# kocvara/Loraine.jl

Measured on AMD Instinct MI355X. Metric: ms/IP-iteration (Schur assembly + solve), dense SDP n=2000 m=4000, lower is better.
Workload: dtype f64; 1 GPU; C4 synthetic dense SDP, matrix side 2000, 4000 constraints, kit=0 (assembly + Cholesky + predictor/corrector solves); msz=2000, nvar=4000, seed=20250614, parallelism=1 GPU

## Files before the change

### loraine.jl_amd/csrc/api.hip

```cpp
#include <cstring>

#include "../../include/loraine_hip.h"
#include "ctx.h"

using namespace lrn;

void lrn_free_model(lrn_ctx* c);
namespace lrn {
void prec_free(lrn_ctx* c);
}

extern "C" {

int lrn_version(void) { return 102; }

int lrn_device_count(void) {
  int n = 0;
  if (hipGetDeviceCount(&n) != hipSuccess) {
    (void)hipGetLastError();
    return 0;
  }
  return n;
}

// ... 58 lines not shown
}

int lrn_set_option(lrn_ctx* c, const char* key, double value) {
  if (!c || !key) return LRN_ERR_ARG;
  if (!strcmp(key, "dense_threshold")) c->opt.dense_threshold = value;
  else if (!strcmp(key, "profile")) c->profile = value != 0.0;
  else if (!strcmp(key, "t_batch")) { c->opt.t_batch = (long)value; for (auto& b : c->lmi) b.t_cap = b.p_cap = 0; }
  else if (!strcmp(key, "p_batch")) { c->opt.p_batch = (long)value; for (auto& b : c->lmi) b.t_cap = b.p_cap = 0; }
  else if (!strcmp(key, "prec_eig")) c->opt.prec_eig = (int)value;
  else if (!strcmp(key, "pivot_boost")) c->opt.pivot_boost = value;
  else if (!strcmp(key, "schur_chol")) c->opt.schur_chol = (int)value;
  else if (!strcmp(key, "schur_plan")) c->opt.schur_plan = (int)value;
  else if (!strcmp(key, "gemm3_ksplit")) c->opt.gemm3_ksplit = (int)value;
  else if (!strcmp(key, "gemm_no_skip")) c->opt.gemm_no_skip = (int)value;
  else if (!strcmp(key, "gemm_dyn_masks")) c->opt.gemm_dyn_masks = (int)value;
  else if (!strcmp(key, "gemm1_diag")) c->opt.gemm1_diag = (int)value;
  else if (!strcmp(key, "gemm_lab")) c->opt.gemm_lab = (int)value & 127;
  else if (!strcmp(key, "gemm3_sched")) c->opt.gemm3_sched = (int)value;
  else if (!strcmp(key, "gemm3_tile")) c->opt.gemm3_tile = (int)value;
  else if (!strcmp(key, "gemm3_strip")) c->opt.gemm3_strip = (int)value;
  else if (!strcmp(key, "gemm3_stagger")) c->opt.gemm3_stagger = (int)value;
  else if (!strcmp(key, "jacobi_wgs")) c->opt.jacobi_wgs = (int)value;
  else if (!strcmp(key, "jacobi_block")) c->opt.jacobi_block = (int)value;
  else if (!strcmp(key, "jacobi_inner")) c->opt.jacobi_inner = (int)value;
  else if (!strcmp(key, "pair_lanes")) c->opt.pair_lanes = (int)value;
  else if (!strcmp(key, "matvec_sparse")) c->opt.matvec_sparse = (int)value;
  else if (!strcmp(key, "prec_dense")) c->opt.prec_dense = (int)value;
  else if (!strcmp(key, "wmw_pattern_min")) c->opt.wmw_pattern_min = std::max(2, (int)value);
  else if (!strcmp(key, "profile_symv")) c->opt.profile_symv = (int)value;
  else if (!strcmp(key, "profile_ops")) c->opt.profile_ops = (int)value;
// ... 461 lines not shown
```

### loraine.jl_amd/csrc/ctx.h

```cpp
#pragma once
#include <map>

#include "chol.h"
#include "lrn_common.h"

namespace lrn { struct Prec; struct Comm; }

struct LmiBlock {
  int msz = 0;
  long nent = 0;
  std::vector<int> sigma;
  std::vector<int> ipos;
  std::vector<long> nnz;
  int qA = 0;
  int nd = 0;
  int q_wave = 0;
  int npos_nz = 0;
  long p_cap = 0, t_cap = 0;
  lrn::DBuf ent_ptr;
  lrn::DBuf ent_r, ent_c;
  lrn::DBuf ent_v;
  lrn::DBuf Adense;
  int dense_sym = -1;
  lrn::DBuf tri_tab;
// ... 34 lines not shown
  bool factored = false;
};

struct lrn_ctx;
namespace lrn { void update_shard_bs(lrn_ctx* c); }

struct LrnOptions {
  double dense_threshold = -1.0;
  long t_batch = 0, p_batch = 0;
  int prec_eig = 0;
  double pivot_boost = 1e-12;
  int schur_chol = -1;
  int schur_plan = -1;
  int gemm3_ksplit = 0;
  int gemm_dyn_masks = 0;
  int gemm_lab = 0;
  int gemm1_diag = 1;
  int gemm_no_skip = 0;
  int gemm3_sched = 1;
  int gemm3_strip = 1;
  int gemm3_tile = 0;
  int gemm3_stagger = 0;
  int jacobi_inner = 0;
  int jacobi_wgs = 0;
  int jacobi_block = 0;
  int jacobi_cross = 1;
  int prepw_streams = 1;
  int lz_resident = 1;
  int eigmin_pair = 2;
  double jacobi_early = 3e-8;
// ... 133 lines not shown
```

### loraine.jl_amd/csrc/gemm_f64.hip

```cpp
#include "lrn_common.h"

#include <algorithm>
#include <map>
#include <mutex>
#include <type_traits>
#include <utility>
#include <vector>

namespace lrn {

static constexpr int BK = 16;
static constexpr int MAX_KSPLIT = 64;

struct GemmParams {
  GemmDesc d;
  int tilesM, tilesN;
  int kchunk;
  int kcols[MAX_KSPLIT + 1];
  int kcols2[MAX_KSPLIT + 1];
  const int2* tile_list;
  const int2* tile_list2;
  int n1, n2;
  int m_org = 0, n_org = 0;
};

#define MFMA_F64_ROW(lane, r) (((lane) >> 4) + 4 * (r))
#define LRN_MFMA_INPLACE(c, a, b) asm volatile("v_mfma_f64_16x16x4_f64 %0, %1, %2, %0" : "+v"(c) : "v"(a), "v"(b))
#define LRN_MFMA_DRAIN() asm volatile("s_nop 15\n\ts_nop 15\n\ts_nop 15" ::: "memory")

template <int BM, bool KC>
__device__ __forceinline__ int lds_idx(int m, int k) {
  return KC ? (m * (BK + 2) + k) : (k * (BM + 16) + m);
}

template <int BM, int BN, bool AKC, bool BKC, bool KSEG, bool EPI>
__global__ __launch_bounds__(256, 2) void gemm_f64_kernel(GemmParams p) {
  constexpr int TM = BM / 32, TN = BN / 32;
  constexpr int EA = BM * BK / 256, EB = BN * BK / 256;
  constexpr int LA = BK * (BM + 16), LB = BK * (BN + 16);
  __shared__ double lds[2 * (LA + LB)];

  const GemmDesc& d = p.d;
  int tm, tn;
// ... 200 lines not shown
          *c = v;
          if (mir) Cg[(long)n * d.sCm + (long)m * d.sCn] = v;
          if (EPI && d.C2) d.C2[(long)n * d.sCm + (long)m * d.sCn] = v;
        }
      }
}

template <int BM, int BN, bool KSEG, bool EPI>
static void launch4(hipStream_t st, const GemmParams& p, bool akc, bool bkc, dim3 grid) {
  if (akc && bkc) hipLaunchKernelGGL((gemm_f64_kernel<BM, BN, true, true, KSEG, EPI>), grid, dim3(256), 0, st, p);
  else if (akc) hipLaunchKernelGGL((gemm_f64_kernel<BM, BN, true, false, KSEG, EPI>), grid, dim3(256), 0, st, p);
  else if (bkc) hipLaunchKernelGGL((gemm_f64_kernel<BM, BN, false, true, KSEG, EPI>), grid, dim3(256), 0, st, p);
  else hipLaunchKernelGGL((gemm_f64_kernel<BM, BN, false, false, KSEG, EPI>), grid, dim3(256), 0, st, p);
}

template <bool EPI, bool DYN>
__global__ __launch_bounds__(256, 2) void gemm_f64_lds_kernel(GemmParams p) {
  constexpr int BM = 128, BN = 128, TM = 4, TN = 4;
  constexpr int LROW = BM + 16;
  constexpr int LA = BK * LROW;
  __shared__ double lds[2 * 2 * LA];
  const GemmDesc& d = p.d;
  int tm, tn;
  {
    int bid = blockIdx.x, nwg = gridDim.x;
    int q = nwg >> 3, r = nwg & 7, xcd = bid & 7;
    int swz = (xcd < r ? xcd * (q + 1) : r * (q + 1) + (xcd - r) * q) + (bid >> 3);
    if ((d.flags & (GEMM_KFROM_N | GEMM_KFROM_M | GEMM_KTO_N | GEMM_KTO_M)) && r == 0) {
      xcd = (xcd + (int)blockIdx.z) & 7;
      swz = xcd * q + (bid >> 3);
    }
// ... 77 lines not shown
#pragma unroll
    for (int kk = 0; kk < BK / 4; ++kk) {
      double fa[TM], fb[TN];
#pragma unroll
      for (int i = 0; i < TM; ++i) fa[i] = sa[(kk * 4 + fk) * LROW + (2 * i + wm) * 16 + fr];
#pragma unroll
      for (int j = 0; j < TN; ++j) fb[j] = sb[(kk * 4 + fk) * LROW + (2 * j + wn) * 16 + fr];
#pragma unroll
      for (int i = 0; i < TM; ++i)
#pragma unroll
        for (int j = 0; j < TN; ++j)
          acc[i][j] = __builtin_amdgcn_mfma_f64_16x16x4f64(fa[i], fb[j], acc[i][j], 0, 0, 0);
    }
    __syncthreads();
  };
  auto step_mask = [&](int kt) __attribute__((always_inline)) -> unsigned {
    unsigned mask = smask;
    const int sn = kt - n0 / BK, sm = kt - m0 / BK;
#pragma unroll
    for (int j = 0; j < TN; ++j) {
      const int bn = 2 * j + wn;
      if ((from_n && sn < bn) || (to_n && sn > bn)) mask &= ~(0x1111u << j);
    }
#pragma unroll
    for (int i = 0; i < TM; ++i) {
      const int bm = 2 * i + wm;
      if ((from_m && sm < bm) || (to_m && sm > bm)) mask &= ~(0xfu << (4 * i));
    }
    return mask;
  };
// ... 91 lines not shown
      else if ((smask & ~0xf731u) == 0u) e[10] = nk;
      else if ((smask & ~0x7777u) == 0u) e[3] = nk;
      else if ((smask & ~0x0fffu) == 0u) e[6] = nk;
    }
#define LRN_PATTERN_LOOP(q, m)                                                             \
    {                                                                                      \
      const int end = e[q] < nk ? e[q] : nk;                                               \
      for (; kt < end; ++kt) static_step(std::integral_constant<unsigned, m>{}, kt);       \
    }
    LRN_PATTERN_LOOP(0, 0x0000u)
    LRN_PATTERN_LOOP(1, 0x1111u) LRN_PATTERN_LOOP(2, 0x3333u) LRN_PATTERN_LOOP(3, 0x7777u)
    LRN_PATTERN_LOOP(4, 0x000fu) LRN_PATTERN_LOOP(5, 0x00ffu) LRN_PATTERN_LOOP(6, 0x0fffu)
    LRN_PATTERN_LOOP(7, 0x08ceu) LRN_PATTERN_LOOP(8, 0x8cefu)
    LRN_PATTERN_LOOP(9, 0x7310u) LRN_PATTERN_LOOP(10, 0xf731u)
#undef LRN_PATTERN_LOOP
    for (; kt < nk; ++kt) fast_step(kt);
  }
  LRN_MFMA_DRAIN();
  if (d.flags & GEMM_LAB_NO_STORE) return;

  const bool x2 = EPI && (d.flags & GEMM_OFFDIAG_X2) && (tm != tn);
  const double alpha = x2 ? 2.0 * d.alpha : d.alpha;
  const bool sq = EPI && (d.flags & GEMM_SQUARE);
  const bool pk = EPI && (d.flags & GEMM_C_PACKED);
  const bool mir = EPI && (d.flags & GEMM_C_MIRROR) && (tm != tn);
  const int pkS = packed_S(d.pk_m);
  const long pkKd = packed_diag_elems(d.pk_m > 0 ? d.pk_m : 1);
  if (pk && !sq) {
    const long S16 = pkS >> 4, kd16 = pkKd >> 4;
    const int qb = (m0 + d.pk_off) >> 4, rbb = (n0 + d.pk_off) >> 4;
#pragma unroll
// ... 145 lines not shown
  if (trace && t == 0) trace[6] = wall_clock64();
  double* __restrict__ Cg = d.C + (long)ks * d.sCs;
#pragma unroll
  for (int i = 0; i < 2; ++i)
#pragma unroll
    for (int j = 0; j < 2; ++j)
#pragma unroll
      for (int r = 0; r < 4; ++r) {
        const int m = m0 + wm * 32 + i * 16 + MFMA_F64_ROW(lane, r);
        const int n = n0 + wn * 32 + j * 16 + fr;
        if (m < d.M && n < d.N) Cg[(long)m * d.sCm + n] = d.alpha * acc[i][j][r];
      }
  if (trace && t == 0) trace[7] = wall_clock64();
}

template <bool FLAT, int TBM, int TBN>
__global__ __launch_bounds__(256, 2) void gemm_f64_kseg_lds_kernel(GemmParams p) {
  constexpr int BM = 32 * TBM, BN = 32 * TBN, TM = TBM, TN = TBN;
  constexpr int LA = BM * BK, LB = BN * BK;
  extern __shared__ double lds[];
  const GemmDesc& d = p.d;
  int tm, tn, ks, bz;
  if (p.n2 >= 0) {
    const int xcd = blockIdx.x & 7, l = blockIdx.x >> 3;
    const int q1 = p.n1 >> 3, q2 = p.n2 >> 3;
    int2 tt;
    if (l < d.ksplit * q1) { ks = l / q1; tt = p.tile_list[xcd * q1 + l % q1]; }
    else { const int l2 = l - d.ksplit * q1; ks = l2 / q2; tt = p.tile_list2[xcd * q2 + l2 % q2]; }
    tm = tt.x;
    tn = tt.y;
    bz = 0;
// ... 86 lines not shown
      for (int j = 0; j < TN; ++j) {
        const int bm = 2 * i + wm, bn = 2 * j + wn;
        bool need = (m0 + 16 * bm < d.M) && (n0 + 16 * bn < d.N);
        if ((diag_lo && bm < bn) || (diag_up && bn < bm)) need = false;
        if (d.flags & GEMM_NO_SKIP) need = true;
        if (need) smask |= 1u << (i * TN + j);
      }
  }
  bool more = FLAT ? left > 0 : segc < segcend;
  if (more) {
    issue(chunk_base(), 0);
    next_chunk();
  }
  __syncthreads();
  int cur = 0;
  if (smask == (1u << (TM * TN)) - 1u) {
    while (more) {
      const bool have_next = FLAT ? left > 0 : segc < segcend;
      if (have_next) {
        issue(chunk_base(), cur ^ 1);
        next_chunk();
      }
      const double* sa = lds + cur * (LA + LB);
      const double* sb = same_panel ? sa : sa + LA;
#pragma unroll
      for (int kk = 0; kk < BK / 4; ++kk) {
        double fa[TM], fb[TN];
        const int k = kk * 4 + fk;
#pragma unroll
        for (int i = 0; i < TM; ++i) {
          int row = (2 * i + wm) * 16 + fr;
// ... 61 lines not shown
        int m = m0 + (2 * i + wm) * 16 + MFMA_F64_ROW(lane, r);
        int n = n0 + (2 * j + wn) * 16 + fr;
        if (m < d.M && n < d.N) Cg[(long)m * d.sCm + (long)n * d.sCn] = d.alpha * acc[i][j][r];
      }
    }
}

static bool kseg_lds_path_ok(const GemmDesc& d) {
  if (d.sAk != 1 || d.sBk != 1 || d.beta != 0.0) return false;
  if ((d.flags & GEMM_KFLAT) ? ((d.kflat_total & 15) || (d.kflat_diag & 15)) : (d.kseg_ld & 15)) return false;
  if ((d.sAm & 1) || (d.sBn & 1) || (d.bA & 1) || (d.bB & 1)) return false;
  if (((uintptr_t)d.A & 15) || ((uintptr_t)d.B & 15)) return false;
  if (d.flags & (GEMM_OFFDIAG_X2 | GEMM_SQUARE | GEMM_SQUARE_BLOCKSUM)) return false;
  return true;
}

static bool lds_path_ok(const GemmDesc& d) {
  if (d.sAm != 1 || d.sBn != 1 || d.ksplit != 1) return false;
  if (d.flags & GEMM_SQUARE_BLOCKSUM) return false;
  static const bool aligned_only = getenv("LRN_LDS_ALIGNED") != nullptr;
  if (d.sAk < d.M || d.sBk < d.N || (aligned_only && ((d.sAk & 1) || (d.sBk & 1)))) return false;
  if (aligned_only && (((uintptr_t)d.A & 15) || ((uintptr_t)d.B & 15) || (d.bA & 1) || (d.bB & 1))) return false;
  if (d.K < 256) return false;
  if ((double)d.K * (double)d.sAk * 8.0 >= 2.0e9 || (double)d.K * (double)d.sBk * 8.0 >= 2.0e9) return false;
  return true;
}

static const int2* get_tile_list(int tilesM, int tilesN, int tri, int* count, int short_sel = 0, bool edge_m = false,
                                 bool edge_n = false, bool diag = false, int korder = 0) {
  struct Key {
// ... 52 lines not shown
}

static thread_local const char* tls_gemm_error = nullptr;
const char* gemm_last_error() { return tls_gemm_error; }
static int gemm_fail(int code, const char* why) { tls_gemm_error = why; return code; }

static int gemm_impl(hipStream_t st, const GemmDesc& din);
static bool big_tile_attr_ok() {
  static bool done[64] = {false}, ok[64] = {false};
  int dev = 0;
  if (hipGetDevice(&dev) != hipSuccess || dev < 0 || dev >= 64) return false;
  if (!done[dev]) {
    ok[dev] = hipFuncSetAttribute((const void*)gemm_f64_kseg_lds_kernel<true, 5, 5>,
                                  hipFuncAttributeMaxDynamicSharedMemorySize, 2 * 2 * 160 * BK * 8) == hipSuccess &&
              hipFuncSetAttribute((const void*)gemm_f64_kseg_lds_kernel<true, 4, 5>,
                                  hipFuncAttributeMaxDynamicSharedMemorySize, 2 * (128 + 160) * BK * 8) == hipSuccess;
    done[dev] = true;
  }
  return ok[dev];
}

#include <map>
#include <mutex>
static double* split_slabs(hipStream_t st, size_t bytes) {
  static std::mutex mu;
  static std::map<std::pair<int, hipStream_t>, std::pair<void*, size_t>> cache;
  int dev = 0;
  if (hipGetDevice(&dev) != hipSuccess) return nullptr;
  std::lock_guard<std::mutex> lk(mu);
  auto& e = cache[{dev, st}];
// ... 51 lines not shown
        out->p = slabs; out->stride = (long)mn; out->n = ks;
        return LRN_OK;
      }
      if (out) { out->p = din.C; out->stride = 0; out->n = 1; }
      return reduce_slabs(st, slabs, (long)mn, ks, din.C, (long)mn, din.beta);
    }
  }
  if (out) { out->p = din.C; out->stride = 0; out->n = 1; }
  const int rc = gemm_impl(st, din);
  if (rc != LRN_OK && !tls_gemm_error) tls_gemm_error = "kernel launch failed";
  return rc;
}

int gemm(hipStream_t st, const GemmDesc& din) { return gemm_maybe_slabs(st, din, nullptr); }
int gemm_slabs(hipStream_t st, const GemmDesc& din, SlabSrc* out) { return gemm_maybe_slabs(st, din, out); }

static int gemm_impl(hipStream_t st, const GemmDesc& din) {
  GemmParams p;
  p.d = din;
  GemmDesc& d = p.d;
  if (d.M <= 0 || d.N <= 0 || d.batch <= 0) return LRN_OK;
  if (d.ksplit < 1) d.ksplit = 1;
  if (d.ksplit > MAX_KSPLIT) return gemm_fail(LRN_ERR_ARG, "gemm: d.ksplit > MAX_KSPLIT");
  long asCm = d.sCm < 0 ? -d.sCm : d.sCm, asCn = d.sCn < 0 ? -d.sCn : d.sCn;
  bool swapped = false;
  if (asCm < asCn) {
    swapped = true;
    if (d.flags & GEMM_KFROM_N) d.flags = (d.flags & ~GEMM_KFROM_N) | GEMM_KFROM_M;
    else if (d.flags & GEMM_KFROM_M) d.flags = (d.flags & ~GEMM_KFROM_M) | GEMM_KFROM_N;
    if (d.flags & GEMM_KTO_N) d.flags = (d.flags & ~GEMM_KTO_N) | GEMM_KTO_M;
// ... 99 lines not shown
    int c1 = 0, c2 = 0;
    p.tile_list = get_tile_list(p.tilesM, p.tilesN, trif, &c1, 1, em, en, dg);
    p.tile_list2 = get_tile_list(p.tilesM, p.tilesN, trif, &c2, 2, em, en, dg);
    if (!p.tile_list || !p.tile_list2) return gemm_fail(LRN_ERR_NOMEM, "gemm: tile list allocation failed");
    p.n1 = c1;
    p.n2 = c2;
    if (c1 + c2 == 0) return LRN_OK;
    if (c1 == 0) { p.tile_list = p.tile_list2; p.n1 = c2; p.n2 = 0; }
    const long wgs = 8L * d.ksplit * ((p.n1 >> 3) + (p.n2 >> 3));
    if (wgs > 0x7fffffffL) return gemm_fail(LRN_ERR_ARG, "gemm: grid too large");
    dim3 grid1((unsigned)wgs, 1, 1);
    if (big) {
      if (!big_tile_attr_ok()) return gemm_fail(LRN_ERR_HIP, "gemm: 80 KB of dynamic LDS refused");
      hipLaunchKernelGGL((gemm_f64_kseg_lds_kernel<true, 5, 5>), grid1, dim3(256), 2 * 2 * 160 * BK * 8, st, p);
    } else {
      hipLaunchKernelGGL((gemm_f64_kseg_lds_kernel<true, 4, 4>), grid1, dim3(256), 2 * 2 * 128 * BK * 8, st, p);
    }
    return hipGetLastError() == hipSuccess ? LRN_OK : LRN_ERR_HIP;
  }
  if (d.tile_class == 4 || d.tile_class == 5) {
    const int rem = d.M % 128;
    if (!kflat || d.batch != 1 || big || d.M != d.N || rem == 0 || rem > 32 || d.M < 288 ||
        (d.flags & (GEMM_TRI_LOWER | GEMM_TRI_UPPER)) != GEMM_TRI_UPPER || !(d.flags & GEMM_DIAG_UPPER) ||
        (d.flags & GEMM_NO_SKIP))
      return gemm_fail(LRN_ERR_ARG, "gemm: tile_class 4 needs the symmetric K-contiguous update with M % 128 in (0, 32]");
    if (!big_tile_attr_ok()) return gemm_fail(LRN_ERR_HIP, "gemm: 80 KB of dynamic LDS refused");
    const int Mm = d.M - 128 - rem, tmain = Mm / 128;
    if (d.tile_class == 4) {
      GemmParams pm = p;
      pm.d.M = Mm; pm.d.N = Mm;
      pm.tilesM = tmain; pm.tilesN = tmain;
      int c1 = 0, c2 = 0;
      pm.tile_list = get_tile_list(tmain, tmain, GEMM_TRI_UPPER, &c1, 1, false, false, true);
      pm.tile_list2 = get_tile_list(tmain, tmain, GEMM_TRI_UPPER, &c2, 2, false, false, true);
      if (!pm.tile_list || !pm.tile_list2) return gemm_fail(LRN_ERR_NOMEM, "gemm: tile list allocation failed");
      pm.n1 = c1;
      pm.n2 = c2;
      if (c1 == 0) { pm.tile_list = pm.tile_list2; pm.n1 = c2; pm.n2 = 0; }
      const long wgs = 8L * d.ksplit * ((pm.n1 >> 3) + (pm.n2 >> 3));
      if (wgs > 0x7fffffffL) return gemm_fail(LRN_ERR_ARG, "gemm: grid too large");
      if (wgs > 0)
        hipLaunchKernelGGL((gemm_f64_kseg_lds_kernel<true, 4, 4>), dim3((unsigned)wgs, 1, 1), dim3(256),
                           2 * 2 * 128 * BK * 8, st, pm);
    } else {
      GemmParams ps = p;
      ps.d.flags &= ~(GEMM_TRI_LOWER | GEMM_TRI_UPPER | GEMM_DIAG_LOWER | GEMM_DIAG_UPPER);
      ps.m_org = 0; ps.n_org = Mm;
      ps.tilesM = tmain + 2; ps.tilesN = 1;
      int cnt = 0;
      ps.tile_list = get_tile_list(tmain + 2, 1, 0, &cnt);
      if (!ps.tile_list || cnt <= 0) return gemm_fail(LRN_ERR_NOMEM, "gemm: tile list allocation failed");
      hipLaunchKernelGGL((gemm_f64_kseg_lds_kernel<true, 4, 5>), dim3(cnt, 1, d.ksplit), dim3(256),
                         2 * (128 + 160) * BK * 8, st, ps);
    }
    return hipGetLastError() == hipSuccess ? LRN_OK : gemm_fail(LRN_ERR_HIP, "gemm: launch failed");
  }
  static const int tile_order = getenv("LRN_TILE_ORDER") ? atoi(getenv("LRN_TILE_ORDER")) : 0;
  const int korder = (tile_order && d.tile_class == 0 && d.batch > 1) ? ((d.flags & GEMM_KFROM_N) ? 1 : (d.flags & GEMM_KFROM_M) ? 2 : 0) : 0;
  p.tile_list = get_tile_list(p.tilesM, p.tilesN, d.flags & (GEMM_TRI_LOWER | GEMM_TRI_UPPER), &ntile, d.tile_class,
                              d.tile_class != 0 && (d.M % BMv) != 0, d.tile_class != 0 && (d.N % BMv) != 0,
                              d.tile_class != 0 && (d.flags & (GEMM_DIAG_LOWER | GEMM_DIAG_UPPER)) != 0, korder);
  if (d.tile_class != 0 && p.tile_list && ntile == 0) return LRN_OK;
  if (!p.tile_list || ntile <= 0) return gemm_fail(LRN_ERR_NOMEM, "gemm: tile list allocation failed");
  (void)tri;
  const bool akc = (d.sAk == 1 && d.sAm != 1);
  const bool bkc = (d.sBk == 1 && d.sBn != 1);
  dim3 grid(ntile, 1, d.batch * d.ksplit);
  if (grid.z > 65535) return gemm_fail(LRN_ERR_ARG, "gemm: grid.z > 65535");
  const bool epi = (d.flags & (GEMM_OFFDIAG_X2 | GEMM_SQUARE | GEMM_SQUARE_BLOCKSUM | GEMM_C_PACKED | GEMM_C_MIRROR)) || d.C2;
  if (d.C2 && (d.M != d.N || d.batch != 1 || d.ksplit != 1 || kseg)) return gemm_fail(LRN_ERR_ARG, "gemm: C2 needs a square, unbatched, unsplit product");
  if (kflat) {
    if (big) {
      if (!big_tile_attr_ok()) return gemm_fail(LRN_ERR_HIP, "gemm: 80 KB of dynamic LDS refused");
      hipLaunchKernelGGL((gemm_f64_kseg_lds_kernel<true, 5, 5>), grid, dim3(256), 2 * 2 * 160 * BK * 8, st, p);
    } else {
      hipLaunchKernelGGL((gemm_f64_kseg_lds_kernel<true, 4, 4>), grid, dim3(256), 2 * 2 * 128 * BK * 8, st, p);
    }
    return hipGetLastError() == hipSuccess ? LRN_OK : LRN_ERR_HIP;
  }
  if (kseg && kseg_lds_path_ok(d)) {
    hipLaunchKernelGGL((gemm_f64_kseg_lds_kernel<false, 4, 4>), grid, dim3(256), 2 * 2 * 128 * BK * 8, st, p);
    return hipGetLastError() == hipSuccess ? LRN_OK : LRN_ERR_HIP;
  }
  if (!small && !kseg && lds_path_ok(d)) {
    const unsigned dyn = (d.flags & GEMM_LAB_ONE_WG) ? 24576u : 0u;
    if (dyn) {
      (void)hipFuncSetAttribute((const void*)gemm_f64_lds_kernel<true, false>, hipFuncAttributeMaxDynamicSharedMemorySize, (int)dyn);
      (void)hipFuncSetAttribute((const void*)gemm_f64_lds_kernel<false, false>, hipFuncAttributeMaxDynamicSharedMemorySize, (int)dyn);
    }
    if (d.flags & GEMM_DYN_MASKS) {
      if (epi) hipLaunchKernelGGL((gemm_f64_lds_kernel<true, true>), grid, dim3(256), 0, st, p);
      else hipLaunchKernelGGL((gemm_f64_lds_kernel<false, true>), grid, dim3(256), 0, st, p);
    } else {
      if (epi) hipLaunchKernelGGL((gemm_f64_lds_kernel<true, false>), grid, dim3(256), dyn, st, p);
      else hipLaunchKernelGGL((gemm_f64_lds_kernel<false, false>), grid, dim3(256), dyn, st, p);
    }
    return hipGetLastError() == hipSuccess ? LRN_OK : LRN_ERR_HIP;
  }
  if (small && mid_mode != 0 && !kseg && !epi && d.batch == 1 && d.beta == 0.0 && d.sAm == 1 && d.sBn == 1 && d.K >= 64 &&
      d.sCn == 1 && d.sAk >= d.M && d.sBk >= d.N && !(d.flags & ~(GEMM_SMALL_TILE | GEMM_TRI_LOWER | GEMM_TRI_UPPER)) &&
      (!tri || (d.M == d.N && d.ksplit > 1)) &&
      (double)d.K * (double)std::max(d.sAk, d.sBk) * 8.0 < 2.0e9) {
    static const char* trace_path = getenv("LRN_MID_TRACE");
    static int trace_launch = 0;
    unsigned long long* tb = nullptr;
    p.n1 = (tri ? p.tilesM * (p.tilesM + 1) / 2 : p.tilesM * p.tilesN) * d.ksplit;
    grid = dim3((unsigned)((p.n1 + 7) & ~7), 1, 1);
    const size_t tw = 8 * (size_t)grid.x * grid.z;
    if (trace_path && ++trace_launch == 40 && hipMalloc(&tb, tw * 8) == hipSuccess) {
      (void)hipMemsetAsync(tb, 0, tw * 8, st);
// ... 98 lines not shown
```

### loraine.jl_amd/csrc/lrn_common.h

```cpp
#pragma once
#include <hip/hip_runtime.h>

#include <cstdint>
#include <cstdio>
#include <cstring>
#include <string>
#include <vector>

#define LRN_OK 0
#define LRN_ERR_ARG (-1)
#define LRN_ERR_HIP (-2)
#define LRN_ERR_STATE (-3)
#define LRN_ERR_NOMEM (-4)

typedef double v4f64 __attribute__((ext_vector_type(4)));

namespace lrn {

__host__ __device__ inline int shard_owner(int blk, int world) {
  int r = blk % world;
  return ((blk / world) & 1) ? world - 1 - r : r;
}
__host__ __device__ inline int shard_global_block(int rank, int lb, int world) {
  return lb * world + ((lb & 1) ? world - 1 - rank : rank);
// ... 19 lines not shown
  GEMM_KTO_N = 1024,
  GEMM_KTO_M = 2048,
  GEMM_C_MIRROR = 4096,
  GEMM_DIAG_LOWER = 8192,
  GEMM_DIAG_UPPER = 16384,
  GEMM_TILE160 = 65536,
  GEMM_DYN_MASKS = 131072,
  GEMM_NO_SKIP = 32768,
  GEMM_DIAG_LOWER_Z = 262144,
  GEMM_LAB_SAME_CHUNK = 1 << 25,
  GEMM_LAB_NO_STORE = 1 << 20,
  GEMM_LAB_NO_KLOOP = 1 << 21,
  GEMM_LAB_NO_LOAD = 1 << 22,
  GEMM_LAB_ONE_WG = 1 << 23,
  GEMM_SQUARE_BLOCKSUM = 1 << 26,
  GEMM_KFLAT = 512,
};

__host__ __device__ inline int packed_S(int m) { return (m + 15) & ~15; }
__host__ __device__ inline long packed_diag_elems(int m) { return 16L * m; }
__host__ __device__ inline long packed_off_base(int c, int S) {
  const long q = c >> 4;
  return 16L * (q * S - 8L * q * (q + 1)) + (long)(c - 16 * q) * (S - 16 * (q + 1));
}
__host__ __device__ inline long packed_total_elems(int m) { return packed_diag_elems(m) + packed_off_base(m, packed_S(m)); }
__host__ __device__ inline long packed_lower_offset(int r, int c, int S, long Kd) {
  const int q = c >> 4;
  if ((r >> 4) == q) return 16L * c + (r - 16 * q);
  return Kd + packed_off_base(c, S) + (r - 16 * (q + 1));
}
// ... 50 lines not shown
```

### loraine.jl_amd/csrc/schur.hip

```cpp
#include <algorithm>

#include "ctx.h"

namespace lrn {

static constexpr int TS = 128;
static constexpr int BK_CHUNK = 16;

__device__ __forceinline__ double wave_sum(double v) {
#pragma unroll
  for (int off = 32; off > 0; off >>= 1) v += __shfl_down(v, off, 64);
  return v;
}

template <int LANES>
__global__ __launch_bounds__(256) void pair_wave_kernel(
    const long* __restrict__ ptr, const int* __restrict__ er, const int* __restrict__ ec,
    const double* __restrict__ ev, const double* __restrict__ W, int msz, int p_lo, int p_hi,
    int p_end, const int* __restrict__ hidx, double* __restrict__ H, int ldh, int rank, int world,
    int bs) {
  constexpr int PER_WG = 256 / LANES;
  const int lane = threadIdx.x & (LANES - 1), grp = threadIdx.x / LANES;
  const int pi = p_lo + blockIdx.y;
  if (pi >= p_hi) return;
// ... 194 lines not shown
}

static constexpr long WG_SLOTS = 512;
static double fill_eff(long wgs) { return (double)wgs / (double)(((wgs + WG_SLOTS - 1) / WG_SLOTS) * WG_SLOTS); }

static int pick_ksplit(long tiles, int max_split) {
  int best = 1;
  double beste = 0.0;
  for (int k = 1; k <= max_split; ++k) {
    if (tiles * k < WG_SLOTS && k < max_split) continue;
    double e = fill_eff(tiles * k);
    if (e >= 0.97) return k;
    if (e > beste) { beste = e; best = k; }
  }
  return best;
}

static long pick_p_batch(int m, long limit) {
  long t1 = (long)((m + 127) / 128) * ((m + 127) / 128);
  long tl = (long)((m + 127) / 128);
  long t2 = tl * (tl + 1) / 2;
  long best = std::min<long>(32, limit);
  double beste = 0.0;
  for (long bsz = std::min<long>(16, limit); bsz <= std::min<long>(96, limit); ++bsz) {
    double e = (2.0 * t1 * fill_eff(t1 * bsz) + (double)t2 * fill_eff(t2 * bsz)) / (2.0 * t1 + t2);
    if (e > beste + 1e-9) { beste = e; best = bsz; }
  }
  return best;
}

// ... 162 lines not shown
  double* T = c->T.as<double>();
  for (int a = 0; a < nd; a += (int)P_cap) {
    const int nb = std::min((int)P_cap, nd - a);
    for (auto& rn : runs) {
      const int c0 = rn.first, c1 = rn.second;
      const long off = (long)c0 + (long)c0 * m;
      const long ldp = ((c1 - c0) + 15) & ~15;
      tic(c);
      GemmDesc g1;
      g1.A = Ad + (long)a * mm + off; g1.sAm = 1; g1.sAk = m; g1.bA = mm;
      g1.B = Ut + off; g1.sBk = m; g1.sBn = 1; g1.bB = 0;
      g1.C = P; g1.sCm = ldp; g1.sCn = 1; g1.bC = p_elems;
      g1.M = g1.K = m - c0; g1.N = c1 - c0; g1.batch = nb;
      g1.flags = GEMM_TRI_LOWER | GEMM_KFROM_N | (c->opt.gemm_no_skip ? GEMM_NO_SKIP : 0) |
                 (c->opt.gemm_dyn_masks ? GEMM_DYN_MASKS : 0) | (c->opt.gemm1_diag ? GEMM_DIAG_LOWER_Z : 0) |
                 ((c->opt.gemm_lab & 15) << 20);
      if (c->opt.gemm_lab & 32) g1.bA = 0;
      if (c->opt.gemm_lab & 16) g1.flags &= ~GEMM_KFROM_N;
      LRN_TRY(gemm(c->stream, g1));
      toc(c, "gemm1");
      tic(c);
      GemmDesc g2;
      g2.A = Ut + off; g2.sAm = 1; g2.sAk = m; g2.bA = 0;
      g2.B = P; g2.sBk = ldp; g2.sBn = 1; g2.bB = p_elems;
      g2.C = T + (long)a * 16; g2.sCm = 1; g2.sCn = m; g2.bC = 16;
      g2.pk_cstride = cstride;
      g2.M = g2.K = m - c0; g2.N = c1 - c0; g2.batch = nb;
      g2.flags = GEMM_TRI_LOWER | GEMM_KFROM_M | GEMM_C_PACKED | (c->opt.gemm_no_skip ? GEMM_NO_SKIP : 0) |
                 (c->opt.gemm_dyn_masks ? GEMM_DYN_MASKS : 0) | ((c->opt.gemm_lab & 15) << 20);
      if (c->opt.gemm_lab & 32) g2.bB = 0;
      if (c->opt.gemm_lab & 16) g2.flags &= ~GEMM_KFROM_M;
      g2.pk_m = m;
      g2.pk_off = c0;
      LRN_TRY(gemm(c->stream, g2));
      toc(c, "gemm2");
    }
  }
  double* H = c->H.as<double>();
  double* Hd = H;
  long ldh = n;
  if (!c->pos_space) {
    LRN_TRY(ensure(c, c->Hd, (size_t)nd * nd * 8, true));
    LRN_HIP(c, hipMemsetAsync(c->Hd.p, 0, (size_t)nd * nd * 8, c->stream));
    Hd = c->Hd.as<double>();
// ... 66 lines not shown
        kb.push_back((int)(r.o0 + no_ * i / nso));
        ke.push_back((int)(r.o0 + no_ * (i + 1) / nso));
      }
    }
    const int nslab = (int)kb.size();
    if (nslab > 0) {
      LRN_TRY(ensure(c, c->slabs, (size_t)nslab * M * N * 8));
      tic(c);
      GemmDesc g3;
      g3.A = T; g3.sAm = 16; g3.sAk = 1;
      g3.B = T; g3.sBk = 1; g3.sBn = 16;
      g3.kflat_cstride = cstride;
      g3.C = c->slabs.as<double>(); g3.sCm = 1; g3.sCn = M;
      g3.M = M; g3.N = N;
      g3.flags = GEMM_TRI_LOWER | GEMM_KFLAT | GEMM_DIAG_LOWER | (c->opt.gemm_no_skip ? GEMM_NO_SKIP : 0) |
                 (t160 ? GEMM_TILE160 : 0) | ((c->opt.gemm_lab & 64) ? GEMM_LAB_SAME_CHUNK : 0);
      g3.kflat_total = Kp; g3.kflat_diag = Kd; g3.kflat_nsd = 1;
      g3.kflat_kb = kb.data(); g3.kflat_ke = ke.data();
      g3.kstagger = c->opt.gemm3_stagger;
      g3.ksplit = nslab; g3.sCs = (long)M * N;
      if (two_launches && c->opt.gemm3_sched == 0) {
        g3.tile_class = 1;
        LRN_TRY(gemm(c->stream, g3));
        toc(c, "gemm3");
        tic(c);
        g3.tile_class = 2;
      } else {
        g3.tile_class = two_launches ? 3 : 0;
        if (two_launches && !t160 && c->opt.gemm3_strip && M >= 288 && M % 128 > 0 && M % 128 <= 32) g3.tile_class = 4;
      }
      LRN_TRY(gemm(c->stream, g3));
// ... 488 lines not shown
```

Measured before the change: 1.014 s.

## Add software-pipelined K-step with register double-buffered fragments for GEMM1/GEMM2

Adds new K-step variants to the LDS GEMM kernels. They prefetch the MFMA fragments into two register buffers, rotating them across K-steps, and spread the next tile's LDS-DMA loads between MFMA instructions. Compiler fences and accumulator pins keep that instruction order fixed. It aims to hide LDS read latency and global-to-LDS load issue behind the f64 MFMA chain. By default the rotate variant is turned on for gemm1 and gemm2 only, while gemm3 stays on the old path. The cost is higher register pressure from the doubled fragment buffers, which could hurt occupancy at launch bounds (256,2).

```diff
diff --git a/loraine.jl_amd/csrc/api.hip b/loraine.jl_amd/csrc/api.hip
--- a/loraine.jl_amd/csrc/api.hip
+++ b/loraine.jl_amd/csrc/api.hip
@@ -96,6 +96,7 @@
   else if (!strcmp(key, "gemm3_ksplit")) c->opt.gemm3_ksplit = (int)value;
   else if (!strcmp(key, "gemm_no_skip")) c->opt.gemm_no_skip = (int)value;
   else if (!strcmp(key, "gemm_dyn_masks")) c->opt.gemm_dyn_masks = (int)value;
+  else if (!strcmp(key, "gemm_kstep")) c->opt.gemm_kstep = std::max(-1, std::min(2, (int)value));
   else if (!strcmp(key, "gemm1_diag")) c->opt.gemm1_diag = (int)value;
   else if (!strcmp(key, "gemm_lab")) c->opt.gemm_lab = (int)value & 127;
   else if (!strcmp(key, "gemm3_sched")) c->opt.gemm3_sched = (int)value;
diff --git a/loraine.jl_amd/csrc/ctx.h b/loraine.jl_amd/csrc/ctx.h
--- a/loraine.jl_amd/csrc/ctx.h
+++ b/loraine.jl_amd/csrc/ctx.h
@@ -72,6 +72,7 @@
   int schur_plan = -1;
   int gemm3_ksplit = 0;
   int gemm_dyn_masks = 0;
+  int gemm_kstep = -1;
   int gemm_lab = 0;
   int gemm1_diag = 1;
   int gemm_no_skip = 0;
diff --git a/loraine.jl_amd/csrc/gemm_f64.hip b/loraine.jl_amd/csrc/gemm_f64.hip
--- a/loraine.jl_amd/csrc/gemm_f64.hip
+++ b/loraine.jl_amd/csrc/gemm_f64.hip
@@ -27,6 +27,8 @@
 #define MFMA_F64_ROW(lane, r) (((lane) >> 4) + 4 * (r))
 #define LRN_MFMA_INPLACE(c, a, b) asm volatile("v_mfma_f64_16x16x4_f64 %0, %1, %2, %0" : "+v"(c) : "v"(a), "v"(b))
 #define LRN_MFMA_DRAIN() asm volatile("s_nop 15\n\ts_nop 15\n\ts_nop 15" ::: "memory")
+#define LRN_KSTEP_FENCE() asm volatile("" ::: "memory")
+#define LRN_ACC_PIN(c) asm volatile("" : "+v"(c))
 
 template <int BM, bool KC>
 __device__ __forceinline__ int lds_idx(int m, int k) {
@@ -257,7 +259,7 @@
   else hipLaunchKernelGGL((gemm_f64_kernel<BM, BN, false, false, KSEG, EPI>), grid, dim3(256), 0, st, p);
 }
 
-template <bool EPI, bool DYN>
+template <bool EPI, bool DYN, int KS>
 __global__ __launch_bounds__(256, 2) void gemm_f64_lds_kernel(GemmParams p) {
   constexpr int BM = 128, BN = 128, TM = 4, TN = 4;
   constexpr int LROW = BM + 16;
@@ -365,6 +367,57 @@
     }
     __syncthreads();
   };
+  auto issue_piece = [&](int kt, int buf, int pc) __attribute__((always_inline)) {
+    double* sa = lds + buf * (2 * LA);
+    const int kr = w + 4 * (pc >> 1);
+    const unsigned krow = (unsigned)(kt * BK + kr);
+    if (pc & 1)
+      __builtin_amdgcn_raw_ptr_buffer_load_lds(rb, (__attribute__((address_space(3))) void*)(sa + LA + kr * LROW), 16,
+                                               (int)(offB + krow * (unsigned)ldb * 8u), 0, 0, 0);
+    else
+      __builtin_amdgcn_raw_ptr_buffer_load_lds(ra, (__attribute__((address_space(3))) void*)(sa + kr * LROW), 16,
+                                               (int)(offA + krow * (unsigned)lda * 8u), 0, 0, 0);
+  };
+  [[maybe_unused]] double pfa[2][TM], pfb[2][TN];
+  auto pfrags = [&](const double* sa, int q) __attribute__((always_inline)) {
+    const double* sb = sa + LA;
+#pragma unroll
+    for (int i = 0; i < TM; ++i) pfa[q & 1][i] = sa[(q * 4 + fk) * LROW + (2 * i + wm) * 16 + fr];
+#pragma unroll
+    for (int j = 0; j < TN; ++j) pfb[q & 1][j] = sb[(q * 4 + fk) * LROW + (2 * j + wn) * 16 + fr];
+  };
+  auto pinned_step = [&](int kt, auto rotc, auto heldc) __attribute__((always_inline)) {
+    constexpr bool ROT = decltype(rotc)::value, HELD = decltype(heldc)::value;
+    constexpr int Q = TM * TN;
+    const int cur = kt & 1;
+    const double* sa = lds + cur * (2 * LA);
+    pfrags(sa, 0);
+    LRN_KSTEP_FENCE();
+    if (!ROT) pfrags(sa, 1);
+    if (ROT && !HELD) {
+      issue_piece(kt + 1, cur ^ 1, 0);
+      issue_piece(kt + 1, cur ^ 1, 1);
+    }
+#pragma unroll
+    for (int n = (ROT && !HELD) ? Q : 0; n < 4 * Q; ++n) {
+      const int v = n / Q, i = (n % Q) / TN, j = n % TN;
+      if (n % Q == 0 && v > 0 && (ROT ? v : v + 1) < 4) pfrags(sa, ROT ? v : v + 1);
+      if (n % 8 == 0) {
+        LRN_KSTEP_FENCE();
+        issue_piece(kt + 1, cur ^ 1, n / 8);
+      }
+      const int b = (ROT ? v + 1 : v) & 1;
+      LRN_MFMA_INPLACE(acc[i][j], pfa[b][i], pfb[b][j]);
+    }
+    LRN_KSTEP_FENCE();
+    __syncthreads();
+  };
+  auto held_tail = [&]() __attribute__((always_inline)) {
+#pragma unroll
+    for (int i = 0; i < TM; ++i)
+#pragma unroll
+      for (int j = 0; j < TN; ++j) LRN_MFMA_INPLACE(acc[i][j], pfa[1][i], pfb[1][j]);
+  };
   auto step_mask = [&](int kt) __attribute__((always_inline)) -> unsigned {
     unsigned mask = smask;
     const int sn = kt - n0 / BK, sm = kt - m0 / BK;
@@ -486,7 +539,20 @@
     LRN_PATTERN_LOOP(7, 0x08ceu) LRN_PATTERN_LOOP(8, 0x8cefu)
     LRN_PATTERN_LOOP(9, 0x7310u) LRN_PATTERN_LOOP(10, 0xf731u)
 #undef LRN_PATTERN_LOOP
-    for (; kt < nk; ++kt) fast_step(kt);
+    if constexpr (KS == 0) {
+      for (; kt < nk; ++kt) fast_step(kt);
+    } else if constexpr (KS == 1) {
+      for (; kt < nk; ++kt) pinned_step(kt, std::false_type{}, std::false_type{});
+    } else if (kt < nk) {
+#pragma unroll
+      for (int i = 0; i < TM; ++i)
+#pragma unroll
+        for (int j = 0; j < TN; ++j) LRN_ACC_PIN(acc[i][j]);
+      LRN_KSTEP_FENCE();
+      pinned_step(kt, std::true_type{}, std::false_type{});
+      for (++kt; kt < nk; ++kt) pinned_step(kt, std::true_type{}, std::true_type{});
+      held_tail();
+    }
   }
   LRN_MFMA_DRAIN();
   if (d.flags & GEMM_LAB_NO_STORE) return;
@@ -662,7 +728,7 @@
   if (trace && t == 0) trace[7] = wall_clock64();
 }
 
-template <bool FLAT, int TBM, int TBN>
+template <bool FLAT, int TBM, int TBN, int KS = 0>
 __global__ __launch_bounds__(256, 2) void gemm_f64_kseg_lds_kernel(GemmParams p) {
   constexpr int BM = 32 * TBM, BN = 32 * TBN, TM = TBM, TN = TBN;
   constexpr int LA = BM * BK, LB = BN * BK;
@@ -779,7 +845,98 @@
   }
   __syncthreads();
   int cur = 0;
-  if (smask == (1u << (TM * TN)) - 1u) {
+  if (KS > 0 && !same_panel && smask == (1u << (TM * TN)) - 1u) {
+    static_assert(KS == 0 || TBM <= TBN, "piece order below");
+    constexpr int Q = TM * TN, NP = TBM + TBN;
+    auto issue_piece = [&](long kb, int buf, int pc) __attribute__((always_inline)) {
+      double* sa = lds + buf * (LA + LB);
+      const bool isb = pc >= 2 * TBM || (pc & 1);
+      const int j = pc >= 2 * TBM ? pc - TBM : pc >> 1;
+      const int r8 = 8 * (w + 4 * j);
+      if (isb)
+        __builtin_amdgcn_global_load_lds((const __attribute__((address_space(1))) void*)(pb[j < TBN ? j : 0] + kb),
+                                         (__attribute__((address_space(3))) void*)(sa + LA + r8 * BK), 16, 0, 0);
+      else
+        __builtin_amdgcn_global_load_lds((const __attribute__((address_space(1))) void*)(pa[j < TBM ? j : 0] + kb),
+                                         (__attribute__((address_space(3))) void*)(sa + r8 * BK), 16, 0, 0);
+    };
+    double pfa[2][TM], pfb[2][TN];
+    auto pfrags = [&](const double* sa, int q) __attribute__((always_inline)) {
+      const double* sb = sa + LA;
+      const int k = q * 4 + fk;
+#pragma unroll
+      for (int i = 0; i < TM; ++i) {
+        const int row = (2 * i + wm) * 16 + fr;
+        pfa[q & 1][i] = sa[row * BK + 2 * ((k >> 1) ^ ((row >> 1) & 7)) + (k & 1)];
+      }
+#pragma unroll
+      for (int j = 0; j < TN; ++j) {
+        const int row = (2 * j + wn) * 16 + fr;
+        pfb[q & 1][j] = sb[row * BK + 2 * ((k >> 1) ^ ((row >> 1) & 7)) + (k & 1)];
+      }
+    };
+    auto pinned_step = [&](long kb, auto rotc, auto heldc, auto dmac) __attribute__((always_inline)) {
+      constexpr bool ROT = decltype(rotc)::value, HELD = decltype(heldc)::value, DMA = decltype(dmac)::value;
+      constexpr int N0 = (ROT && !HELD) ? Q : 0;
+      const double* sa = lds + cur * (LA + LB);
+      pfrags(sa, 0);
+      if (DMA) {
+#pragma unroll
+        for (int pc = 0; pc < (N0 + 7) / 8; ++pc) issue_piece(kb, cur ^ 1, pc);
+      }
+#pragma unroll
+      for (int n = N0; n < 4 * Q; ++n) {
+        const int v = n / Q, i = (n % Q) / TN, j = n % TN;
+        if (n % Q == 8 && (ROT ? v > 0 : v < 3)) {
+          LRN_KSTEP_FENCE();
+          pfrags(sa, ROT ? v : v + 1);
+        }
+        if (n % 8 == 0 || n == N0) {
+          LRN_KSTEP_FENCE();
+          if (DMA && n % 8 == 0 && n / 8 < NP) issue_piece(kb, cur ^ 1, n / 8);
+        }
+        const int b = (ROT ? v + 1 : v) & 1;
+        LRN_MFMA_INPLACE(acc[i][j], pfa[b][i], pfb[b][j]);
+      }
+      LRN_KSTEP_FENCE();
+      __syncthreads();
+      cur ^= 1;
+    };
+    static_assert(KS == 0 || FLAT, "the pinned K-step walks flat chunks");
+    const long kb0 = lab_kb >= 0 ? lab_kb : 0, kbs = lab_kb >= 0 ? 0 : d.kflat_cstride;
+    auto next_kb = [&]() __attribute__((always_inline)) -> long {
+      const long kb = kb0 + (long)segc * kbs;
+      next_chunk();
+      return kb;
+    };
+    if (more) {
+#pragma unroll
+      for (int i = 0; i < TM; ++i)
+#pragma unroll
+        for (int j = 0; j < TN; ++j) LRN_ACC_PIN(acc[i][j]);
+      LRN_KSTEP_FENCE();
+      bool have_next = FLAT ? left > 0 : segc < segcend;
+      if constexpr (KS == 1) {
+        while (have_next) {
+          pinned_step(next_kb(), std::false_type{}, std::false_type{}, std::true_type{});
+          have_next = FLAT ? left > 0 : segc < segcend;
+        }
+      } else if (have_next) {
+        pinned_step(next_kb(), std::true_type{}, std::false_type{}, std::true_type{});
+        have_next = FLAT ? left > 0 : segc < segcend;
+        while (have_next) {
+          pinned_step(next_kb(), std::true_type{}, std::true_type{}, std::true_type{});
+          have_next = FLAT ? left > 0 : segc < segcend;
+        }
+#pragma unroll
+        for (int i = 0; i < TM; ++i)
+#pragma unroll
+          for (int j = 0; j < TN; ++j) LRN_MFMA_INPLACE(acc[i][j], pfa[1][i], pfb[1][j]);
+      }
+      pinned_step(0, std::false_type{}, std::false_type{}, std::false_type{});
+      LRN_MFMA_DRAIN();
+    }
+  } else if (smask == (1u << (TM * TN)) - 1u) {
     while (more) {
       const bool have_next = FLAT ? left > 0 : segc < segcend;
       if (have_next) {
@@ -871,6 +1028,8 @@
   if (d.flags & (GEMM_OFFDIAG_X2 | GEMM_SQUARE | GEMM_SQUARE_BLOCKSUM)) return false;
   return true;
 }
+
+static int kstep_of(int flags) { return (flags & GEMM_KSTEP_ROTATE) ? 2 : ((flags & GEMM_KSTEP_SPREAD) ? 1 : 0); }
 
 static bool lds_path_ok(const GemmDesc& d) {
   if (d.sAm != 1 || d.sBn != 1 || d.ksplit != 1) return false;
@@ -953,6 +1112,10 @@
     ok[dev] = hipFuncSetAttribute((const void*)gemm_f64_kseg_lds_kernel<true, 5, 5>,
                                   hipFuncAttributeMaxDynamicSharedMemorySize, 2 * 2 * 160 * BK * 8) == hipSuccess &&
               hipFuncSetAttribute((const void*)gemm_f64_kseg_lds_kernel<true, 4, 5>,
+                                  hipFuncAttributeMaxDynamicSharedMemorySize, 2 * (128 + 160) * BK * 8) == hipSuccess &&
+              hipFuncSetAttribute((const void*)gemm_f64_kseg_lds_kernel<true, 4, 5, 1>,
+                                  hipFuncAttributeMaxDynamicSharedMemorySize, 2 * (128 + 160) * BK * 8) == hipSuccess &&
+              hipFuncSetAttribute((const void*)gemm_f64_kseg_lds_kernel<true, 4, 5, 2>,
                                   hipFuncAttributeMaxDynamicSharedMemorySize, 2 * (128 + 160) * BK * 8) == hipSuccess;
     done[dev] = true;
   }
@@ -1034,6 +1197,16 @@
 
 int gemm(hipStream_t st, const GemmDesc& din) { return gemm_maybe_slabs(st, din, nullptr); }
 int gemm_slabs(hipStream_t st, const GemmDesc& din, SlabSrc* out) { return gemm_maybe_slabs(st, din, out); }
+
+template <int TBM, int TBN>
+static void launch_kflat(hipStream_t st, const GemmParams& p, dim3 grid) {
+  const unsigned ldsb = 2 * 32 * (TBM + TBN) * BK * 8;
+  switch (kstep_of(p.d.flags)) {
+    case 2: hipLaunchKernelGGL((gemm_f64_kseg_lds_kernel<true, TBM, TBN, 2>), grid, dim3(256), ldsb, st, p); break;
+    case 1: hipLaunchKernelGGL((gemm_f64_kseg_lds_kernel<true, TBM, TBN, 1>), grid, dim3(256), ldsb, st, p); break;
+    default: hipLaunchKernelGGL((gemm_f64_kseg_lds_kernel<true, TBM, TBN, 0>), grid, dim3(256), ldsb, st, p);
+  }
+}
 
 static int gemm_impl(hipStream_t st, const GemmDesc& din) {
   GemmParams p;
@@ -1163,7 +1336,7 @@
       if (!big_tile_attr_ok()) return gemm_fail(LRN_ERR_HIP, "gemm: 80 KB of dynamic LDS refused");
       hipLaunchKernelGGL((gemm_f64_kseg_lds_kernel<true, 5, 5>), grid1, dim3(256), 2 * 2 * 160 * BK * 8, st, p);
     } else {
-      hipLaunchKernelGGL((gemm_f64_kseg_lds_kernel<true, 4, 4>), grid1, dim3(256), 2 * 2 * 128 * BK * 8, st, p);
+      launch_kflat<4, 4>(st, p, grid1);
     }
     return hipGetLastError() == hipSuccess ? LRN_OK : LRN_ERR_HIP;
   }
@@ -1189,8 +1362,7 @@
       const long wgs = 8L * d.ksplit * ((pm.n1 >> 3) + (pm.n2 >> 3));
       if (wgs > 0x7fffffffL) return gemm_fail(LRN_ERR_ARG, "gemm: grid too large");
       if (wgs > 0)
-        hipLaunchKernelGGL((gemm_f64_kseg_lds_kernel<true, 4, 4>), dim3((unsigned)wgs, 1, 1), dim3(256),
-                           2 * 2 * 128 * BK * 8, st, pm);
+        launch_kflat<4, 4>(st, pm, dim3((unsigned)wgs, 1, 1));
     } else {
       GemmParams ps = p;
       ps.d.flags &= ~(GEMM_TRI_LOWER | GEMM_TRI_UPPER | GEMM_DIAG_LOWER | GEMM_DIAG_UPPER);
@@ -1199,8 +1371,7 @@
       int cnt = 0;
       ps.tile_list = get_tile_list(tmain + 2, 1, 0, &cnt);
       if (!ps.tile_list || cnt <= 0) return gemm_fail(LRN_ERR_NOMEM, "gemm: tile list allocation failed");
-      hipLaunchKernelGGL((gemm_f64_kseg_lds_kernel<true, 4, 5>), dim3(cnt, 1, d.ksplit), dim3(256),
-                         2 * (128 + 160) * BK * 8, st, ps);
+      launch_kflat<4, 5>(st, ps, dim3(cnt, 1, d.ksplit));
     }
     return hipGetLastError() == hipSuccess ? LRN_OK : gemm_fail(LRN_ERR_HIP, "gemm: launch failed");
   }
@@ -1223,7 +1394,7 @@
       if (!big_tile_attr_ok()) return gemm_fail(LRN_ERR_HIP, "gemm: 80 KB of dynamic LDS refused");
       hipLaunchKernelGGL((gemm_f64_kseg_lds_kernel<true, 5, 5>), grid, dim3(256), 2 * 2 * 160 * BK * 8, st, p);
     } else {
-      hipLaunchKernelGGL((gemm_f64_kseg_lds_kernel<true, 4, 4>), grid, dim3(256), 2 * 2 * 128 * BK * 8, st, p);
+      launch_kflat<4, 4>(st, p, grid);
     }
     return hipGetLastError() == hipSuccess ? LRN_OK : LRN_ERR_HIP;
   }
@@ -1234,15 +1405,22 @@
   if (!small && !kseg && lds_path_ok(d)) {
     const unsigned dyn = (d.flags & GEMM_LAB_ONE_WG) ? 24576u : 0u;
     if (dyn) {
-      (void)hipFuncSetAttribute((const void*)gemm_f64_lds_kernel<true, false>, hipFuncAttributeMaxDynamicSharedMemorySize, (int)dyn);
-      (void)hipFuncSetAttribute((const void*)gemm_f64_lds_kernel<false, false>, hipFuncAttributeMaxDynamicSharedMemorySize, (int)dyn);
-    }
+      (void)hipFuncSetAttribute((const void*)gemm_f64_lds_kernel<true, false, 0>, hipFuncAttributeMaxDynamicSharedMemorySize, (int)dyn);
+      (void)hipFuncSetAttribute((const void*)gemm_f64_lds_kernel<false, false, 0>, hipFuncAttributeMaxDynamicSharedMemorySize, (int)dyn);
+    }
+    const int ks = dyn ? 0 : kstep_of(d.flags);
     if (d.flags & GEMM_DYN_MASKS) {
-      if (epi) hipLaunchKernelGGL((gemm_f64_lds_kernel<true, true>), grid, dim3(256), 0, st, p);
-      else hipLaunchKernelGGL((gemm_f64_lds_kernel<false, true>), grid, dim3(256), 0, st, p);
+      if (epi) hipLaunchKernelGGL((gemm_f64_lds_kernel<true, true, 0>), grid, dim3(256), 0, st, p);
+      else hipLaunchKernelGGL((gemm_f64_lds_kernel<false, true, 0>), grid, dim3(256), 0, st, p);
+    } else if (ks == 2) {
+      if (epi) hipLaunchKernelGGL((gemm_f64_lds_kernel<true, false, 2>), grid, dim3(256), 0, st, p);
+      else hipLaunchKernelGGL((gemm_f64_lds_kernel<false, false, 2>), grid, dim3(256), 0, st, p);
+    } else if (ks == 1) {
+      if (epi) hipLaunchKernelGGL((gemm_f64_lds_kernel<true, false, 1>), grid, dim3(256), 0, st, p);
+      else hipLaunchKernelGGL((gemm_f64_lds_kernel<false, false, 1>), grid, dim3(256), 0, st, p);
     } else {
-      if (epi) hipLaunchKernelGGL((gemm_f64_lds_kernel<true, false>), grid, dim3(256), dyn, st, p);
-      else hipLaunchKernelGGL((gemm_f64_lds_kernel<false, false>), grid, dim3(256), dyn, st, p);
+      if (epi) hipLaunchKernelGGL((gemm_f64_lds_kernel<true, false, 0>), grid, dim3(256), dyn, st, p);
+      else hipLaunchKernelGGL((gemm_f64_lds_kernel<false, false, 0>), grid, dim3(256), dyn, st, p);
     }
     return hipGetLastError() == hipSuccess ? LRN_OK : LRN_ERR_HIP;
   }
diff --git a/loraine.jl_amd/csrc/lrn_common.h b/loraine.jl_amd/csrc/lrn_common.h
--- a/loraine.jl_amd/csrc/lrn_common.h
+++ b/loraine.jl_amd/csrc/lrn_common.h
@@ -57,6 +57,8 @@
   GEMM_LAB_NO_LOAD = 1 << 22,
   GEMM_LAB_ONE_WG = 1 << 23,
   GEMM_SQUARE_BLOCKSUM = 1 << 26,
+  GEMM_KSTEP_SPREAD = 1 << 27,
+  GEMM_KSTEP_ROTATE = 1 << 28,
   GEMM_KFLAT = 512,
 };
 
diff --git a/loraine.jl_amd/csrc/schur.hip b/loraine.jl_amd/csrc/schur.hip
--- a/loraine.jl_amd/csrc/schur.hip
+++ b/loraine.jl_amd/csrc/schur.hip
@@ -232,6 +232,12 @@
     if (e > beste) { beste = e; best = k; }
   }
   return best;
+}
+
+static constexpr int KSTEP_DEFAULT[4] = {0, 2, 2, 0};
+static int kstep_flags(const lrn_ctx* c, int which) {
+  const int v = c->opt.gemm_kstep >= 0 ? c->opt.gemm_kstep : KSTEP_DEFAULT[which];
+  return v >= 2 ? (GEMM_KSTEP_SPREAD | GEMM_KSTEP_ROTATE) : (v == 1 ? GEMM_KSTEP_SPREAD : 0);
 }
 
 static long pick_p_batch(int m, long limit) {
@@ -424,7 +430,7 @@
       g1.M = g1.K = m - c0; g1.N = c1 - c0; g1.batch = nb;
       g1.flags = GEMM_TRI_LOWER | GEMM_KFROM_N | (c->opt.gemm_no_skip ? GEMM_NO_SKIP : 0) |
                  (c->opt.gemm_dyn_masks ? GEMM_DYN_MASKS : 0) | (c->opt.gemm1_diag ? GEMM_DIAG_LOWER_Z : 0) |
-                 ((c->opt.gemm_lab & 15) << 20);
+                 ((c->opt.gemm_lab & 15) << 20) | kstep_flags(c, 1);
       if (c->opt.gemm_lab & 32) g1.bA = 0;
       if (c->opt.gemm_lab & 16) g1.flags &= ~GEMM_KFROM_N;
       LRN_TRY(gemm(c->stream, g1));
@@ -437,7 +443,7 @@
       g2.pk_cstride = cstride;
       g2.M = g2.K = m - c0; g2.N = c1 - c0; g2.batch = nb;
       g2.flags = GEMM_TRI_LOWER | GEMM_KFROM_M | GEMM_C_PACKED | (c->opt.gemm_no_skip ? GEMM_NO_SKIP : 0) |
-                 (c->opt.gemm_dyn_masks ? GEMM_DYN_MASKS : 0) | ((c->opt.gemm_lab & 15) << 20);
+                 (c->opt.gemm_dyn_masks ? GEMM_DYN_MASKS : 0) | ((c->opt.gemm_lab & 15) << 20) | kstep_flags(c, 2);
       if (c->opt.gemm_lab & 32) g2.bB = 0;
       if (c->opt.gemm_lab & 16) g2.flags &= ~GEMM_KFROM_M;
       g2.pk_m = m;
@@ -534,7 +540,7 @@
       g3.C = c->slabs.as<double>(); g3.sCm = 1; g3.sCn = M;
       g3.M = M; g3.N = N;
       g3.flags = GEMM_TRI_LOWER | GEMM_KFLAT | GEMM_DIAG_LOWER | (c->opt.gemm_no_skip ? GEMM_NO_SKIP : 0) |
-                 (t160 ? GEMM_TILE160 : 0) | ((c->opt.gemm_lab & 64) ? GEMM_LAB_SAME_CHUNK : 0);
+                 (t160 ? GEMM_TILE160 : 0) | ((c->opt.gemm_lab & 64) ? GEMM_LAB_SAME_CHUNK : 0) | kstep_flags(c, 3);
       g3.kflat_total = Kp; g3.kflat_diag = Kd; g3.kflat_nsd = 1;
       g3.kflat_kb = kb.data(); g3.kflat_ke = ke.data();
       g3.kstagger = c->opt.gemm3_stagger;
```

Result: no change. 1.022 s (+0.8%).
